# TravisWheelerLab/BATH

Hardware: AMD Instinct MI355X
Metric: DP Gcells/s + residues/s through bathsearch pipeline at 1/2/4/8 MI355X (higher is better)
Workload: dtype u8/i16 integer scores (SSV: exact binary16), f32 Forward

## Files before the change

bath_amd/__init__.py:

```python
import ctypes as C
import os
import subprocess

import numpy as np

_HERE = os.path.dirname(os.path.abspath(__file__))
_ROOT = os.path.dirname(_HERE)
LIB_PATH = os.environ.get("BATH_HIP_LIBRARY") or os.path.join(_HERE, "libbathhip.so")

OK, EINVAL, ERANGE, ENORESULT = 0, 11, 16, 19
KP, K, NEVPARAM = 29, 20, 8
LOGSUM_TABLE, LOGSUM_EXACT, LOGSUM_TABLE_SERIAL, LOGSUM_CONTEXT = 0, 1, 2, 3
LOGSUM_ODDS = 4
ENSEMBLE_SERIAL, ENSEMBLE_STREAMS_HOST, ENSEMBLE_STREAMS_DEVICE = 0, 1, 2
ENSEMBLE_MODES = {"serial": ENSEMBLE_SERIAL, "streams": ENSEMBLE_STREAMS_HOST, "device": ENSEMBLE_STREAMS_DEVICE}
ENS_SAMPLES = 200
ARITH_STRICT, ARITH_ODDS3, ARITH_ODDS = 0, 1, 2
ARITH_MODES = {"strict": ARITH_STRICT, "odds3": ARITH_ODDS3, "odds": ARITH_ODDS}
ENS_OK, ENS_IMPOSSIBLE, ENS_STEP_CAP, ENS_SEG_OVERFLOW = 0, 1, 2, 3
ENS_REGION_OK, ENS_REGION_NO_TRACES = 0, 1

DNA_SYMS = "ACGT-RYMKSWHBVDN*~"
AMINO_SYMS = "ACDEFGHIKLMNPQRSTVWY-BJZOUX*~"

# ... 249 lines not shown
    "bath_hits_count": (C.c_int64, [_vp]),
    "bath_hits_domains": (C.POINTER(FsDomain), [_vp]),
    "bath_hits_cigars": (C.c_void_p, [_vp, _i64p]),
    "bath_hits_traces": (C.c_int, [_vp, C.POINTER(C.POINTER(DomainTrace)), C.POINTER(C.POINTER(C.c_int8)), C.POINTER(_i32p), C.POINTER(_i32p),
                                   C.POINTER(C.POINTER(C.c_int8)), C.POINTER(_f32p)]),
    "bath_tophits_add_serialized": (C.c_int, [_vp, C.c_void_p, C.c_int64, C.c_int64, C.c_int64, C.c_int64, C.POINTER(C.c_char_p), C.POINTER(C.c_char_p),
                                              C.POINTER(C.c_char_p), C.POINTER(C.c_int64)]),
    "bath_dist_shard_range": (None, [C.c_int64, C.c_int, C.c_int, _i64p, _i64p]),
    "bath_dist_items": (C.c_int64, [_i64p, C.POINTER(C.c_double), C.c_int, C.c_int, C.c_int, C.POINTER(DistItem), C.c_int64]),
    "bath_dist_deal": (C.c_int, [C.POINTER(C.c_double), C.c_int64, C.c_int, _i32p]),
    "bath_selftest_cluster_segments": (C.c_int, [C.c_int, _i32p, _i32p, _i32p, _i32p, _i32p, C.c_int, C.c_int, _i32p, C.c_int, _i32p]),
    "bath_selftest_fs_ensemble": (C.c_int, [C.c_int, _f32p, C.c_float, C.c_float, C.c_float, C.c_int, C.c_int, _f32p, _f32p, _i32p, C.c_int, _i32p]),
    "bath_tophits_create": (_vp, []),
    "bath_tophits_destroy": (None, [_vp]),
    "bath_tophits_add": (C.c_int, [_vp, C.POINTER(FsDomain), C.c_int64, C.c_void_p, C.c_int64, C.POINTER(C.c_char_p), C.POINTER(C.c_char_p),
                                   C.POINTER(C.c_char_p), C.POINTER(C.c_int64)]),
    "bath_tophits_finalize": (C.c_int, [_vp, C.c_int64, C.c_int, C.c_double]),
    "bath_tophits_count": (C.c_int64, [_vp]),
    "bath_tophits_reported": (C.c_int64, [_vp]),
    "bath_tophits_get": (C.c_int, [_vp, C.c_int64, C.POINTER(FsDomain), C.POINTER(C.c_int64), C.POINTER(C.c_int32)]),
    "bath_tophits_targets": (C.c_int64, [_vp, C.c_int, C.c_int, C.c_char_p, C.c_int64]),
    "bath_tophits_domain_annotation": (C.c_int64, [_vp, C.c_int64, C.c_int, C.c_int, C.c_char_p, C.c_int64]),
    "bath_tophits_pipeline_statistics": (C.c_int64, [_vp, C.POINTER(PipelineStats), C.POINTER(PipelineParams), C.c_int64, C.c_int64, C.c_int64, C.c_char_p, C.c_int64]),
    "bath_tophits_set_inclusion": (None, [_vp, C.c_double]),
    "bath_tophits_tabular_targets": (C.c_int64, [_vp, C.c_char_p, C.c_char_p, C.c_int, C.c_int, C.c_int, C.c_int, C.c_char_p, C.c_int64]),
    "bath_trace_frameshift_rows": (C.c_int64, [C.POINTER(DomainTrace), C.POINTER(C.c_int8), _i32p, _i32p, C.POINTER(C.c_int8), _u8p, C.c_int32,
                                               C.POINTER(_FsProfile), C.c_int64, C.c_int64, C.POINTER(FsRow), C.c_int64]),
    "bath_tophits_tabular_frameshifts": (C.c_int64, [_vp, C.c_char_p, C.c_char_p, C.POINTER(FsRow), _i64p, C.c_int64, C.c_int, C.c_char_p, C.c_int64]),
    "bath_hip_pipeline_hits": (C.c_int, [_vp, _vp, _vp, C.POINTER(PipelineParams), C.c_double, C.POINTER(PipelineStats),
                                         C.POINTER(C.POINTER(FsDomain)), C.POINTER(C.c_int64), C.POINTER(C.c_int64)]),
    "bath_hip_pipeline_frameshift_domains": (C.c_int, [_vp, _vp, _vp, _vp, _vp, C.POINTER(PipelineParams), C.c_double, C.POINTER(PipelineStats),
                                                      C.POINTER(C.POINTER(FsWindow)), _i64p, C.POINTER(C.POINTER(FsDomain)), _i64p, _i64p]),
    "bath_hip_pipeline_timings": (C.c_int, [_vp, C.c_int, C.POINTER(C.c_char_p), _f32p, _i64p]),
    "bath_hip_fsprofile_convert": (C.c_int, [_vp, C.POINTER(_FsProfile), C.POINTER(_vp)]),
    "bath_hip_fsprofile_destroy": (None, [_vp]),
    "bath_hip_fs3_forward_parser": (C.c_int, [_vp, _vp, _vp, C.c_int, _f32p, _f32p, _i64p]),
    "bath_hip_fs3_backward_parser": (C.c_int, [_vp, _vp, _vp, C.c_int, _f32p, _f32p, _i64p]),
    "bath_hip_vitfilter_bath": (C.c_int, [_vp, _vp, _vp, _f32p, C.c_double, _f32p, _i32p, C.POINTER(C.POINTER(HmmWindow)), _i64p]),
    "bath_hip_ssvfilter_bath": (C.c_int, [_vp, _vp, _vp, C.c_double, C.POINTER(C.POINTER(HmmWindow)), _i64p]),
    "bath_hip_forward_full": (C.c_int, [_vp, _vp, _vp, _i32p, C.c_int, _f32p, _i32p, _f32p, _f32p]),
    "bath_hip_std_envelopes": (C.c_int, [_vp, _vp, _vp, C.POINTER(StdResult), _f32p, _f32p, _f32p, _f32p]),
    "bath_hip_std_envelopes_fill": (C.c_int, [_vp, _vp, _vp, C.POINTER(StdResult), _f32p, _f32p, _f32p, _f32p, C.c_int]),
    "bath_hip_fs5_envelopes_x": (C.c_int, [_vp, _vp, _vp, C.c_int, C.c_int, C.POINTER(Fs5Result), _f32p, _f32p, _f32p, _f32p]),
    "bath_hip_fs5_forward_full": (C.c_int, [_vp, _vp, _vp, C.c_int, _f32p, _f32p, _f32p]),
    "bath_hip_fs5_envelopes": (C.c_int, [_vp, _vp, _vp, C.c_int, C.c_int, C.POINTER(Fs5Result), _f32p, _i64p, _f32p, _i64p]),
    "bath_hip_fs5_forward_parser": (C.c_int, [_vp, _vp, _vp, C.c_int, _f32p]),
    "bath_hip_fs5_forward_parser_odds": (C.c_int, [_vp, _vp, _vp, C.c_int, _f32p]),
    "bath_calib_fit_scores": (C.c_int, [C.POINTER(C.c_uint32), _f32p, C.c_int, C.c_int, C.c_int, _CALIB_SCORE_FN, C.c_void_p, C.c_float,
                                        C.POINTER(C.c_double), C.POINTER(C.c_int)]),
    "bath_hip_calibrate_fs_arith": (C.c_int, [_vp, C.POINTER(_Hmm), C.c_int, C.POINTER(C.c_uint32), C.c_int, C.c_int, C.c_double,
                                              C.POINTER(C.c_double), C.POINTER(C.c_double), C.POINTER(C.c_double), C.POINTER(C.c_double),
                                              C.c_int, C.POINTER(C.c_int)]),
    "bath_calib_sample": (C.c_int, [C.POINTER(C.c_uint32), _f32p, C.c_int, C.c_int, C.c_int, _u8p]),
    "bath_gumbel_fit_complete": (C.c_int, [C.POINTER(C.c_double), C.c_int, C.POINTER(C.c_double), C.POINTER(C.c_double)]),
    "bath_gumbel_invcdf": (C.c_double, [C.c_double, C.c_double, C.c_double]),
    "bath_calib_tau": (C.c_int, [C.POINTER(C.c_double), C.c_int, C.c_double, C.c_double, C.POINTER(C.c_double)]),
    "bath_bg_fs_nullone": (C.c_float, [C.c_int]),
    "bath_hmm_max_length": (C.c_int, [C.POINTER(_Hmm), C.c_double]),
    "bath_hip_calibrate_fs": (C.c_int, [_vp, C.POINTER(_Hmm), C.c_int, C.POINTER(C.c_uint32), C.c_int, C.c_int, C.c_double,
                                        C.POINTER(C.c_double), C.POINTER(C.c_double), C.POINTER(C.c_double), C.POINTER(C.c_double)]),
    "bath_calib_sample_batch": (C.c_int, [C.POINTER(C.c_uint32), _f32p, C.POINTER(C.c_int), C.c_int, C.c_int, C.c_int, _u8p]),
    "bath_hip_calibrate_fs_batch": (C.c_int, [_vp, C.POINTER(C.POINTER(_Hmm)), C.POINTER(C.c_int), C.c_int, C.POINTER(C.c_uint32), C.c_int, C.c_int,
                                              C.c_double, C.POINTER(C.c_double), C.POINTER(C.c_double), C.POINTER(C.c_double), C.POINTER(C.c_double)]),
    "bath_scorematrix_builtin": (C.c_char_p, [C.c_char_p]),
    "bath_scoresystem_create": (C.c_int, [C.c_char_p, C.c_char_p, C.c_double, C.c_double, C.POINTER(_vp), C.c_char_p, C.c_int]),
    "bath_scoresystem_destroy": (None, [_vp]),
# ... 266 lines not shown
            offsets = np.zeros(len(seqs) + 1, dtype=np.int64)
            np.cumsum(lens, out=offsets[1:])
            flat = np.concatenate([np.asarray(s, dtype=np.uint8) for s in seqs]) if len(seqs) else np.zeros(0, np.uint8)
        else:
            flat = np.ascontiguousarray(seqs, dtype=np.uint8)
            offsets = np.ascontiguousarray(offsets, dtype=np.int64)
        if flat.size == 0:
            flat = np.zeros(1, np.uint8)
        self.n = len(offsets) - 1
        self.lengths = np.diff(offsets)
        h = _vp()
        ctx._check(lib().bath_hip_seqs_create(ctx._h, _u8(flat), _i64(offsets), self.n, C.byref(h)), "seqs_create")
        self.ctx, self._h = ctx, h

    def set_context(self, context):
        if context is None:
            self.ctx._check(lib().bath_hip_seqs_set_context(self._h, None), "seqs_set_context")
            return
        c = np.ascontiguousarray(context, dtype=np.int32)
        assert c.shape == (self.n,)
        self.ctx._check(lib().bath_hip_seqs_set_context(self._h, c.ctypes.data_as(C.POINTER(C.c_int32))), "seqs_set_context")

    def read(self):
        L = lib()
        nbytes = L.bath_hip_seqs_read(self._h, None, 0, None, None, None)
        if nbytes < 0:
            self.ctx._check(-1, "seqs_read")
        data = np.zeros(nbytes, np.uint8)
        off, ln, cx = np.zeros(max(self.n, 1), np.int64), np.zeros(max(self.n, 1), np.int32), np.zeros(max(self.n, 1), np.int32)
        if L.bath_hip_seqs_read(self._h, _u8(data), nbytes, _i64(off), ln.ctypes.data_as(_i32p), cx.ctypes.data_as(_i32p)) != nbytes:
            self.ctx._check(-1, "seqs_read")
        return data, off[:self.n], ln[:self.n], cx[:self.n]

    def __del__(self):
        if getattr(self, "_h", None) and getattr(self.ctx, "_h", None):
            lib().bath_hip_seqs_destroy(self._h)
        self._h = None


def pack2(flat, offsets):
    flat = np.ascontiguousarray(flat, dtype=np.uint8)
    offsets = np.ascontiguousarray(offsets, dtype=np.int64)
    lens = np.diff(offsets)
    n = len(lens)
    bad = np.flatnonzero(flat[offsets[0]:offsets[-1]] > 3) + offsets[0]
    seq = np.searchsorted(offsets, bad, side="right") - 1
    pos = (bad - offsets[seq]).astype(np.int32)
    codes = flat[bad].copy()
    if n and (lens == lens[0]).all() and lens[0] % 4 == 0:
        q = (flat[offsets[0]:offsets[-1]] & 3).reshape(-1, 4)
        packed = (q[:, 0] | (q[:, 1] << 2) | (q[:, 2] << 4) | (q[:, 3] << 6)).astype(np.uint8)
    else:
        parts = []
        for i in range(n):
            s = flat[offsets[i]:offsets[i + 1]] & 3
            pad = (-len(s)) % 4
            q = np.concatenate([s, np.zeros(pad, np.uint8)]).reshape(-1, 4)
            parts.append((q[:, 0] | (q[:, 1] << 2) | (q[:, 2] << 4) | (q[:, 3] << 6)).astype(np.uint8))
        packed = np.concatenate(parts) if parts else np.zeros(0, np.uint8)
    return packed, seq.astype(np.int64), pos, codes


class PinnedBuffer:

    def __init__(self, nbytes):
        self.ptr = lib().bath_hip_host_alloc(max(int(nbytes), 1))
# ... 1130 lines not shown
```

bath_amd/csrc/bath_common.hpp:

```cpp
#pragma once
#include <set>
#include <atomic>
#include <hip/hip_runtime.h>

#include <cstdint>
#include <chrono>
#include <cstdio>
#include <cstdlib>
#include <cstring>
#include <condition_variable>
#include <functional>
#include <mutex>
#include <string>
#include <thread>
#include <vector>

#include "bath_hip.h"
#include "bath_tilings.hpp"
#include "bath_slots.hpp"

namespace bath {

inline hipError_t allow_max_lds(const void *fn) {
  static std::mutex mu;
// ... 95 lines not shown
    cv_done.wait(l, [&] { return pending == 0; });
  }
  ~LanePool() {
    { std::lock_guard<std::mutex> l(m); stop = true; }
    cv_work.notify_all();
    for (std::thread &t : th) t.join();
  }
};

struct StageTiming { const char *name; float ms; int64_t launches; };
struct KernelSpan { const char *name; hipEvent_t a, b; double cells, bytes; };

struct PipelineSurvivor {
  int64_t window;
  int64_t aa_off;
  int32_t strand, start;
  int32_t n;
  int32_t win_start = 0;
  int32_t fs_window = -1;
  int64_t fx_off = -1;
};

}

struct bath_hip_ctx;
namespace bath {
extern std::atomic<int> g_ctx_total, g_ctx_internal;
inline int host_contexts() { return g_ctx_total.load() - g_ctx_internal.load(); }
inline void mark_internal(bath_hip_ctx *c);
}
struct bath_hip_ctx {
  int device = 0;
  hipStream_t stream = nullptr;
  hipStream_t tail_stream = nullptr;
  hipStream_t side_stream = nullptr;
  hipEvent_t ev_fork = nullptr, ev_join = nullptr;
  hipStream_t copy_stream = nullptr;
  hipDeviceProp_t prop{};
  int fs_strict = 1;
  int fs_odds = 0;
  int fs5_odds = 0;
  int fs_ensemble = 0;
  std::atomic<int64_t> fs_ens_bound_fallbacks{0}, fs_ens_overflow_fallbacks{0}, fs_ens_bytes_kept{0};
  int std_ensemble = 0;
  std::atomic<int64_t> std_ens_serial_fallbacks{0}, std_ens_twin_fallbacks{0}, std_ens_kernel_regions{0};
  int fs_serial = -1;
  uint64_t tabs_uid = 0;
  const void *tabs_ptr = nullptr;
  uint64_t fsw_pad_uid = 0;
  int orf_tables_id = -1;
  std::string err;
  void set_error(const std::string &m) { err = m; }
  std::vector<float> fsw_len_terms;
  bath::SlotArray<bath::Scratch, bath::DevBuf> scratch;
  bath::SlotArray<bath::Pinned, bath::HostBuf> stage;
  template <class T> int stage_upload(bath::Pinned slot, void *dst, const T *src, size_t n, hipStream_t s) {
    if (stage[slot].reserve(n * sizeof(T) + 64) != hipSuccess) { set_error("cannot allocate page-locked staging memory"); return BATH_EFAIL; }
    std::memcpy(stage[slot].p, src, n * sizeof(T));
    if (hipMemcpyAsync(dst, stage[slot].p, n * sizeof(T), hipMemcpyHostToDevice, s) != hipSuccess) { set_error("staging upload failed"); return BATH_EFAIL; }
    return BATH_OK;
  }
  bath::HostBuf pinned[4];
  bath::HostBuf results_pinned;
  bath_orf_result *d_records = nullptr;
  int64_t n_records = 0;
  std::vector<bath_orf> orfs;
  std::vector<bath_fs_window> fs_windows;
// ... 44 lines not shown
  }
  void span_end(int idx, hipStream_t s) { if (idx >= 0) (void)hipEventRecord(spans[(size_t)idx].b, s); }
  std::vector<bath_hip_ctx *> lanes;
  bath::LanePool *lane_pool = nullptr;
  hipEvent_t ev_lanes = nullptr;
  bath_hip_ctx *aux = nullptr;
  bath_hip_ctx *aux2 = nullptr;
  bath_hip_ctx *aux3 = nullptr;
  bool internal = false;
};

namespace bath {
inline void mark_internal(bath_hip_ctx *c) { if (c && !c->internal) { c->internal = true; g_ctx_internal.fetch_add(1); } }
}

struct SeqView {
  const uint8_t *data;
  const int64_t *off;
  const int32_t *len;
  int64_t n;
  const int32_t *context;
};

struct bath_hip_seqs {
  bath_hip_ctx *ctx = nullptr;
  int64_t n = 0;
  int64_t total = 0;
  int64_t total_aligned = 0;
  mutable int64_t cache_minlen = -1, cache_nres = 0, cache_max_orfs = 0;
  mutable int64_t ntiles = -1;
  mutable void *d_tile_desc = nullptr;
  mutable int32_t *d_tile_first = nullptr;
  bool is_part = false;
  int64_t first_window = 0;
  mutable std::vector<bath_hip_seqs *> parts;
  int32_t maxlen = 0;
  uint8_t *d_data = nullptr;
  int64_t *d_off = nullptr;
  int32_t *d_len = nullptr;
  int32_t *d_context = nullptr;
  uint8_t *d_packed = nullptr;
  int64_t *d_poff = nullptr;
  int64_t packed_bytes = 0;
  void *d_exc = nullptr;
  int64_t exc_cap = 0, n_exc = 0;
  hipEvent_t ev_upload = nullptr;
  bool upload_pending = false;
  std::vector<int64_t> h_off;
  std::vector<int32_t> h_len;
  std::vector<int32_t> h_context;
  SeqView view() const { return SeqView{d_data, d_off, d_len, n, d_context}; }
};

struct LenTables {
  int32_t maxL = -1;
  uint8_t *d_tjb = nullptr;
  int16_t *d_xwmove = nullptr;
  float   *d_pmove = nullptr;
  float   *d_nullsc = nullptr;
  float   *d_lt1 = nullptr;
  float   *d_lt2 = nullptr;
  float   *d_p1 = nullptr;
  std::vector<uint8_t> h_tjb;
  std::vector<int16_t> h_xwmove;
  std::vector<float> h_pmove, h_nullsc;
};
// ... 66 lines not shown
```

bath_amd/csrc/bath_launch.hpp:

```cpp
#pragma once
#include <utility>

#include "bath_common.hpp"

namespace bath {

struct Cand {
  int64_t *window;  int32_t *sf;
  int32_t *startj;  int32_t *len;
  int16_t *v;
  int64_t *off;
  int32_t *msv_status, *vit_status, *fwd_status, *stage, *flags;
  float *usc, *nullsc, *filtersc, *vfsc, *fwdsc;
  double *P;
  int32_t *kminmax;
};

int build_orf_records(bath_hip_ctx *ctx, const Cand &cand, int nc, int64_t window_offset, bath_orf_result **d_out, int64_t *n_out);

struct VitWindowArgs {
  double invP_vit, invP_msv;
  const float *d_filtersc;
  const uint8_t *d_ssv_scores;
  void *d_wins;
  int *d_win_count;
  int win_cap;
  int32_t *d_kminmax;
};

int ssv_table_fits(bath_hip_ctx *ctx, const bath_hip_oprofile *om);
int launch_ssv_lane(bath_hip_ctx *ctx, const bath_hip_oprofile *om, SeqView v, const int32_t *d_order, int16_t *d_v);
int launch_ssv_classify(bath_hip_ctx *ctx, const bath_hip_oprofile *om, int64_t n, const int32_t *d_len, const int16_t *d_v, float *d_sc, int32_t *d_status);
int launch_msv_wave(bath_hip_ctx *ctx, const bath_hip_oprofile *om, SeqView v, const int32_t *d_todo, int64_t ntodo, float *d_sc, int32_t *d_status, const int *ntodo_dev, bool lane_ok = true);
int launch_msv_lane(bath_hip_ctx *ctx, const bath_hip_oprofile *om, SeqView v, const int32_t *d_todo, int64_t ntodo, float *d_sc, int32_t *d_status, const int *ntodo_dev);
bool msv_stage_supported(const bath_hip_oprofile *om);
int launch_vit_wave(bath_hip_ctx *ctx, const bath_hip_oprofile *om, SeqView v, const int32_t *d_todo, int64_t ntodo, float *d_sc, int32_t *d_status,
                    const VitWindowArgs *wa, const int *ntodo_dev);
int launch_fwd_wave(bath_hip_ctx *ctx, const bath_hip_oprofile *om, SeqView v, const int32_t *d_todo, int64_t ntodo, float *d_sc, int32_t *d_status, const int *ntodo_dev,
                    float *d_xmx = nullptr, const int64_t *d_xmx_off = nullptr, float *d_dp = nullptr, const int64_t *d_dp_off = nullptr, int unihit = 0,
                    const int32_t *d_cfg_len = nullptr);
int launch_bwd_wave(bath_hip_ctx *ctx, const bath_hip_oprofile *om, SeqView v, int64_t n, const float *d_fwd_xmx, const int64_t *d_xmx_off,
                    float *d_sc, int32_t *d_status, float *d_bck_xmx, float *d_dp = nullptr, const int64_t *d_dp_off = nullptr, int unihit = 0);
int launch_bias_lane(bath_hip_ctx *ctx, const bath_hip_oprofile *om, SeqView v, const float *d_eo, int eo_stride, const int32_t *d_todo, int64_t ntodo,
                     float *d_nullsc, float *d_filtersc);

int vit_lane_supported(const bath_hip_oprofile *om);
int launch_len_sort(bath_hip_ctx *ctx, const int32_t *d_todo, const int *d_ntodo, const int32_t *d_len, int *d_bins, int32_t *d_sorted);
int launch_vit_lane(bath_hip_ctx *ctx, const bath_hip_oprofile *om, SeqView v, const int32_t *d_todo, int64_t ntodo, const int *ntodo_dev,
                    float *d_sc, int32_t *d_status, const VitWindowArgs *wa, const int *skip_dev = nullptr);
const int *len_sort_count_longer(const int *d_bins, int T);
int64_t lane_min_nt();
const char *vit_lane_kernel_name(const bath_hip_oprofile *om);
int launch_vit_sorted(bath_hip_ctx *ctx, const bath_hip_oprofile *om, SeqView v, const int32_t *d_todo, int64_t cap, const int *d_ntodo, const int32_t *d_len,
                      int *d_bins, int32_t *d_sorted, float *d_sc, int32_t *d_status, const VitWindowArgs *wa, const std::function<int(hipStream_t)> &beside);
struct MsvConsts;
MsvConsts msv_consts(const bath_hip_oprofile *om);

int pipeline_filters_survivors(bath_hip_ctx *ctx, const bath_hip_oprofile *om, const bath_hip_seqs *dna, const bath_pipeline_params *prm,
                               bath_pipeline_stats *stats, std::vector<PipelineSurvivor> *out, const uint8_t **d_pool);

struct FsWinDev {
  int64_t src_off;
  int64_t dst_off;
  int32_t seq_n, start, len, strand, kmin, kmax;
};
int fs_gather_view(bath_hip_ctx *ctx, const bath_hip_seqs *dna, std::vector<FsWinDev> &regs, const uint8_t *d_comp, bath_hip_seqs *view, const FsWinDev **d_desc_out);

struct WindowRec;
struct FsCandRec { int64_t window, aa_off; double P; int32_t cand, sf, startj, len; float fwdsc, nullsc; int64_t fxoff; };
struct FsLaneSurv {
  const FsCandRec *d_c; const WindowRec *d_w;
  int32_t n_c, n_w, cand_base;
  int64_t first_window, dpool;
};
struct FsOrfDev {
  int64_t w, aa_off; double P;
  int32_t cand, strand, start, end, n; float fwd_null;
  int32_t wb, we;
  int32_t dw_n, dw_len, dw_k;
  int32_t kmin, kmax;
  int32_t g0, g1;
  int32_t pad_;
};
struct FsWinBuild {
  int32_t n_orfs = 0, nw = 0, maxlen = 0;
// ... 120 lines not shown
```

bath_amd/csrc/bath_pipeline.hip:

```cpp
#include <algorithm>
#include <cmath>
#include <cstring>
#include <cstdlib>
#include <map>
#include <thread>

#include "bath_common.hpp"
#include "bath_kernels.hpp"
#include "bath_launch.hpp"
#include "host_model.hpp"

using namespace bath;

namespace bath {

static const double kLog2 = 0.69314718055994529;

enum { FLAG_VIT_RUN = 1, FLAG_HAS_WIN = 2 };

struct Counters {
  int cand_count, todo_msv, todo_vit, todo_ssvb, todo_vit2, todo_fwd, win_count, overflow;
  int todo_lb, pad_;
  unsigned long long n_orfs, orf_res;
  unsigned long long n_past_msv, n_past_bias, n_past_vit, n_past_fwd;
  unsigned long long pos_past_msv, pos_past_bias, pos_past_vit, pos_past_fwd;
  unsigned long long res_vit, res_fwd;
  unsigned long long res_seen;
};

struct Params {
  double F1, F2, F3, F4;
  int do_bias, fs_pipe, minlen;
  float evparam[BATH_NEVPARAM];
};

template <int NR, int G>
__global__ __launch_bounds__(256, NR <= 76 ? 4 : 1) void ssv_orf_kernel(const uint8_t *__restrict__ aa, const OrfRec *__restrict__ orfs, const int *__restrict__ n_orfs_dev,
                                                      SeqView dna, const int16_t *__restrict__ cost_tab, int row_bytes,
// ... 662 lines not shown
struct FilterState {
  PipelineWork W;
  Counters hc{};
  const uint8_t *d_ssvsc = nullptr;
  const float *d_bgf = nullptr;
  OrfTablesDev tt{};
};
}

__global__ __launch_bounds__(64) void fwd_keep_offsets_kernel(const int32_t *__restrict__ todo, const int *__restrict__ ntodo_dev, const int32_t *__restrict__ len,
                                                              int64_t *__restrict__ off, int64_t cap) {
  const int lane = threadIdx.x, n = *ntodo_dev;
  int64_t base = 0;
  for (int j0 = 0; j0 < n; j0 += 64) {
    const int j = j0 + lane;
    const int sid = j < n ? todo[j] : -1;
    const int64_t v = sid >= 0 ? ((int64_t)len[sid] + 1) * 6 : 0;
    int64_t incl = v;
    for (int d = 1; d < 64; d <<= 1) { const int64_t u = __shfl_up(incl, d, 64); if (lane >= d) incl += u; }
    if (sid >= 0) off[sid] = (base + incl <= cap) ? base + incl - v : (int64_t)-1;
    base += __shfl(incl, 63, 64);
  }
}

static int cascade_model_ok(bath_hip_ctx *ctx, const bath_hip_oprofile *om) {
  if (om->M <= kCascadeMaxNodes) return BATH_OK;
  ctx->set_error("the filter cascade supports models up to " + std::to_string(kCascadeMaxNodes) + " nodes (this one has " + std::to_string(om->M) + ")");
  return BATH_EINVAL;
}

static int launch_ssv_bath(bath_hip_ctx *ctx, hipStream_t stream, const bath_hip_oprofile *om, const Cand &cand, Counters *ctr, const int32_t *todo, const uint8_t *pool,
                           const uint8_t *ssv_scores, const MsvConsts &mc, double invP, WindowRec *wins, int win_cap);

static int run_filters(bath_hip_ctx *ctx, const bath_hip_oprofile *om, const bath_hip_seqs *dna,
                       const bath_pipeline_params *prm, bath_pipeline_stats *stats,
                       const bath_orf_result **results, int64_t *n_results, FilterState *state) {
  if (!ctx || !om || !dna || !prm) return BATH_EINVAL;
  if (cascade_model_ok(ctx, om) != BATH_OK) return BATH_EINVAL;
  BATH_HIP_TRY(ctx, hipSetDevice(ctx->device));
  if (n_results) *n_results = 0;
  if (results) *results = nullptr;
  if (stats) std::memset(stats, 0, sizeof *stats);
  const int64_t nwin = dna->n;
  if (nwin == 0) return BATH_OK;
  const int M = om->M;
  const int max_orf = dna->maxlen / 3 + 1;
  int st = om->ensure_len_tables(max_orf);
  if (st != BATH_OK) return st;

  OrfTablesDev tt{};
  if (prm->strands < 0 || prm->strands > 2 || prm->initiator < 0 || prm->initiator > 2) { ctx->set_error("bath_pipeline_params: strands / initiator out of range"); return BATH_EINVAL; }
  if ((st = orf_tables_upload(ctx, prm->ncbi_table, &tt, prm->initiator)) != BATH_OK) return st;
  if ((st = ensure_emit_table(ctx, om, prm->F1, max_orf)) != BATH_OK) return st;
  DevBuf &b_tabs = ctx->scratch[Scratch::kSsvScoreTable], &b_work = ctx->scratch[Scratch::kCascadeWork];
  const size_t ssv_bytes = (size_t)(M + 1) * kKp;
  const size_t tabs_bytes = 8192 + ssv_bytes + 256 + 20 * 4 + 256;
  if (tabs_bytes > b_tabs.cap) ctx->tabs_uid = 0;
  BATH_HIP_TRY(ctx, b_tabs.reserve(tabs_bytes));
  char *tp = b_tabs.as<char>();
  const int16_t *d_emit = om->d_emit;
  uint8_t *d_ssvsc = reinterpret_cast<uint8_t *>(tp); tp += (ssv_bytes + 255) / 256 * 256;
  float *d_bgf = reinterpret_cast<float *>(tp);
  if (ctx->tabs_uid != om->uid || ctx->tabs_ptr != b_tabs.p) {
    std::vector<uint8_t> ssv_scores(ssv_bytes, 0);
    bath_hip_oprofile_get_ssv_scores(om, ssv_scores.data());
    BATH_HIP_TRY(ctx, hipMemcpyAsync(d_ssvsc, ssv_scores.data(), ssv_scores.size(), hipMemcpyHostToDevice, ctx->stream));
// ... 40 lines not shown
  BATH_HIP_TRY(ctx, b_orfs.reserve((size_t)(max_orfs + 64) * sizeof(OrfRec)));
  BATH_HIP_TRY(ctx, b_misc.reserve((5 * nent + kOrfMiscInts) * sizeof(int32_t)));
  OrfBuffers ob{};
  orf_buffers_carve(&ob, b_aa.p, b_slots.p, b_orfs.p, b_misc.p, nent);

  const int NRk = om->NR;
  const size_t ssv_shmem = (size_t)kSsvRows * om->ssv_row_bytes;
  if ((st = ssv_table_fits(ctx, om)) != BATH_OK) return st;
  const int dec_blocks = ctx->prop.multiProcessorCount * 4;

  std::vector<hipEvent_t> &ev = ctx->ev_pool;
  while (ev.size() < 12) { hipEvent_t e; BATH_HIP_TRY(ctx, hipEventCreate(&e)); ev.push_back(e); }

  PipelineWork W;
  Counters hc{};
  int win_need = 0;
  for (int attempt = 0;; attempt++) {
    size_t need = layout(W, nullptr, (int)cap, win_need);
    BATH_HIP_TRY(ctx, b_work.reserve(need + 4096));
    layout(W, b_work.as<char>(), (int)cap, win_need);
    W.pool = b_aa.as<uint8_t>();
    BATH_HIP_TRY(ctx, hipMemsetAsync(W.ctr, 0, sizeof(Counters), ctx->stream));
    SeqView cv{W.pool, W.cand.off, W.cand.len, cap};

    int e = 0;
    BATH_HIP_TRY(ctx, hipEventRecord(ev[e++], ctx->stream));
    if ((st = launch_orf_scan(ctx, dna, tt, prm->min_orf_len, ob, &W.ctr->n_orfs, &W.ctr->orf_res, prm->strands)) != BATH_OK) return st;
    BATH_HIP_TRY(ctx, hipEventRecord(ev[e++], ctx->stream));
    {
      static const int ssv_chunk = [] { const char *e = std::getenv("BATH_HIP_SSV_CHUNK"); return e ? std::atoi(e) : 0; }();
      int blocks = ctx->prop.multiProcessorCount * 4;
      const int ssv_threads = 256;
      const int wpb = ssv_threads / 64;
      if (ssv_chunk > 0) blocks = (int)std::min<int64_t>((max_orfs + (int64_t)wpb * (64 / om->G) * ssv_chunk - 1) / ((int64_t)wpb * (64 / om->G) * ssv_chunk), 1 << 30);
      bool launched = false;
#define BATH_ORF_CASE(N, GG)                                                                                                     \
  if (!launched && NRk == N && om->G == GG) {                                                                                    \
    if (ssv_shmem > 64 * 1024) (void)bath::allow_max_lds((const void *)ssv_orf_kernel<N, GG>); \
    hipLaunchKernelGGL((ssv_orf_kernel<N, GG>), dim3(blocks), dim3(ssv_threads), ssv_shmem, ctx->stream, W.pool, ob.sorted, ob.ntotal,                  \
                       dna->view(), om->d_ssv, om->ssv_row_bytes, d_emit, max_orf, W.cand, W.cand_cap, W.ctr, ssv_chunk);        \
    launched = true;                                                                                                             \
  }
      BATH_SSV_SHAPES(BATH_ORF_CASE)
#undef BATH_ORF_CASE
      if (!launched) { ctx->set_error("SSV kernel: no tile shape for this model length"); return BATH_EINVAL; }
      BATH_HIP_TRY(ctx, hipGetLastError());
    }
    BATH_HIP_TRY(ctx, hipEventRecord(ev[e++], ctx->stream));
    hipStream_t bulk_stream = ctx->stream;
    struct StreamRestore { bath_hip_ctx *c; hipStream_t s; ~StreamRestore() { c->stream = s; } } stream_restore{ctx, bulk_stream};
    if (ctx->tail_stream) {
      BATH_HIP_TRY(ctx, hipStreamWaitEvent(ctx->tail_stream, ev[e - 1], 0));
      ctx->stream = ctx->tail_stream;
    }
    const bool few_cands = dna->total < lane_min_nt(), few_msv = dna->total < 2 * lane_min_nt();
    const F1Tables f1t{om->d_bias_eo, om->lt.d_nullsc, om->lt.d_p1, om->lt.d_lt1, om->lt.d_lt2};
    const bool msv_stage = !few_msv && msv_stage_supported(om);
    if (msv_stage) {
      bool launched = false;
#define BATH_MSV_STAGE_CASE(N, ...)                                                                                                         \
  if (!launched && NRk == N) {                                                                                                              \
    hipLaunchKernelGGL((msv_stage_kernel<N>), dim3((unsigned)((W.cand_cap + 255) / 256)), dim3(256), ssv_shmem, ctx->stream, W.cand, W.cand_cap, W.ctr, om->d_msv, \
                       om->ssv_row_bytes, om->lt.d_tjb, mc, P, W.pool, M, f1t, W.todo_vit, W.todo_ssvb);                                      \
    launched = true;                                                                                                                        \
  }
      BATH_MSV_LANE_NR(BATH_MSV_STAGE_CASE)
#undef BATH_MSV_STAGE_CASE
      if (!launched) { ctx->set_error("MSV stage kernel: no tile shape for this model length"); return BATH_EINVAL; }
      BATH_HIP_TRY(ctx, hipGetLastError());
      BATH_HIP_TRY(ctx, hipEventRecord(ev[e++], ctx->stream));
      BATH_HIP_TRY(ctx, hipEventRecord(ev[e++], ctx->stream));
// ... 67 lines not shown
      BATH_HIP_TRY(ctx, hipEventElapsedTime(&ms, ev[i], ev[i + 1]));
      ctx->timings.push_back(StageTiming{names[i], ms, launches[i]});
    }
    break;
  }

  if (stats) {
    stats->nres = nres; stats->n_orfs = (int64_t)hc.n_orfs;
    stats->n_past_msv = (int64_t)hc.n_past_msv; stats->n_past_bias = (int64_t)hc.n_past_bias;
    stats->n_past_vit = (int64_t)hc.n_past_vit; stats->n_past_fwd = (int64_t)hc.n_past_fwd;
    stats->pos_past_msv = (int64_t)hc.pos_past_msv; stats->pos_past_bias = (int64_t)hc.pos_past_bias;
    stats->pos_past_vit = (int64_t)hc.pos_past_vit; stats->pos_past_fwd = (int64_t)hc.pos_past_fwd;
    stats->cells_msv = (int64_t)(hc.orf_res - hc.res_seen) * M; stats->cells_vit = (int64_t)hc.res_vit * M; stats->cells_fwd = (int64_t)hc.res_fwd * M;
  }

  if (results) {
    bath_orf_result *d_rec = nullptr;
    int64_t nrec = 0;
    if (dna->n > (int64_t)UINT32_MAX || dna->maxlen / 3 >= (1 << 28)) { ctx->set_error("block too large for the ORF records' sort key (2^32 windows, 805 Mnt per window)"); return BATH_ERANGE; }
    if ((st = build_orf_records(ctx, W.cand, hc.cand_count, dna->is_part ? dna->first_window : 0, &d_rec, &nrec)) != BATH_OK) return st;
    ctx->d_records = d_rec; ctx->n_records = nrec;
    if (!dna->is_part) {
      BATH_HIP_TRY(ctx, ctx->results_pinned.reserve((size_t)std::max<int64_t>(nrec, 1) * sizeof(bath_orf_result)));
      if (nrec > 0) BATH_HIP_TRY(ctx, hipMemcpyAsync(ctx->results_pinned.p, d_rec, (size_t)nrec * sizeof(bath_orf_result), hipMemcpyDeviceToHost, ctx->stream));
      BATH_HIP_TRY(ctx, hipStreamSynchronize(ctx->stream));
      *results = ctx->results_pinned.as<bath_orf_result>();
    } else *results = nullptr;
    if (n_results) *n_results = nrec;
  } else if (n_results) *n_results = (int64_t)hc.n_past_msv;
  if (state) { state->W = W; state->hc = hc; state->d_ssvsc = d_ssvsc; state->d_bgf = d_bgf; state->tt = tt; }
  return BATH_OK;
}

static int pipeline_lane_count(const bath_hip_seqs *dna) {
  const char *e = std::getenv("BATH_HIP_LANES");
  const int forced = e ? std::atoi(e) : 0;
  if (forced > 0) return (int)std::min<int64_t>(forced, std::max<int64_t>(dna->n, 1));
  if (dna->is_part || dna->n < 8) return 1;
  int K = (dna->total >= ((int64_t)1 << 28)) ? 2 : 1;
  const int64_t by_size = (dna->total + ((int64_t)1 << 34) - 1) >> 34;
  if (by_size > K) K = (int)std::min<int64_t>(by_size, std::max<int64_t>(dna->n, 1));
  return K;
}

static int ensure_parts(bath_hip_ctx *ctx, const bath_hip_seqs *dna, int K) {
  if ((int)dna->parts.size() == K) return BATH_OK;
  for (bath_hip_seqs *p : dna->parts) bath_hip_seqs_destroy(p);
  dna->parts.clear();
  int64_t w0 = 0;
  for (int k = 0; k < K; k++) {
    static const double split2 = [] { const char *e = std::getenv("BATH_HIP_LANE_SPLIT"); const double v = e ? std::atof(e) : 0.0; return (v > 0.05 && v < 0.95) ? v : 0.5; }();
    int64_t w1 = w0;
    if (k == K - 1) w1 = dna->n;
    else {
      const int64_t target = (K == 2) ? (int64_t)((double)dna->total_aligned * split2) : dna->total_aligned / K * (k + 1);
      w1 = std::lower_bound(dna->h_off.begin() + w0, dna->h_off.end(), target) - dna->h_off.begin();
      w1 = std::max(w1, std::min(w0 + 1, dna->n));
    }
    bath_hip_seqs *p = new bath_hip_seqs();
    p->ctx = ctx; p->is_part = true; p->first_window = w0; p->n = w1 - w0;
    const int64_t base = w0 < dna->n ? dna->h_off[(size_t)w0] : dna->total_aligned;
    p->h_off.resize((size_t)p->n); p->h_len.assign(dna->h_len.begin() + w0, dna->h_len.begin() + w1);
    for (int64_t i = 0; i < p->n; i++) {
      p->h_off[(size_t)i] = dna->h_off[(size_t)(w0 + i)] - base;
      p->maxlen = std::max(p->maxlen, p->h_len[(size_t)i]);
      p->total += p->h_len[(size_t)i];
    }
    p->total_aligned = (w1 < dna->n ? dna->h_off[(size_t)w1] : dna->total_aligned) - base;
    p->d_data = dna->d_data + base;
    p->d_len = dna->d_len + w0;
    if (dna->d_context) { p->d_context = dna->d_context + w0; p->h_context.assign(dna->h_context.begin() + w0, dna->h_context.begin() + w1); }
    dna->parts.push_back(p);
    if (hipMalloc((void **)&p->d_off, (size_t)std::max<int64_t>(p->n, 1) * sizeof(int64_t)) != hipSuccess) { ctx->set_error("hipMalloc (block parts)"); return BATH_EMEM; }
    if (p->n > 0 && hipMemcpy(p->d_off, p->h_off.data(), (size_t)p->n * sizeof(int64_t), hipMemcpyHostToDevice) != hipSuccess) { ctx->set_error("hipMemcpy (block parts)"); return BATH_EFAIL; }
    w0 = w1;
  }
  return BATH_OK;
}

template <class After>
static int run_filters_lanes(bath_hip_ctx *ctx, const bath_hip_oprofile *om, const bath_hip_seqs *dna,
                             const bath_pipeline_params *prm, bath_pipeline_stats *stats,
                             const bath_orf_result **results, int64_t *n_results, std::vector<FilterState> *states, After after) {
  if (!ctx || !om || !dna || !prm) return BATH_EINVAL;
  if (cascade_model_ok(ctx, om) != BATH_OK) return BATH_EINVAL;
  const int K = pipeline_lane_count(dna);
  if (K <= 1) {
    states->assign(1, FilterState{});
    int st = run_filters(ctx, om, dna, prm, stats, results, n_results, &(*states)[0]);
    if (st != BATH_OK) return st;
    return after(0, ctx, dna, (*states)[0]);
  }
  BATH_HIP_TRY(ctx, hipSetDevice(ctx->device));
  int st = om->ensure_len_tables(dna->maxlen / 3 + 1);
  if (st != BATH_OK) return st;
  if ((st = ensure_emit_table(ctx, om, prm->F1, dna->maxlen / 3 + 1)) != BATH_OK) return st;
  while ((int)ctx->lanes.size() < K) {
    bath_hip_ctx *lane = nullptr;
    if ((st = bath_hip_init(ctx->device, &lane)) != BATH_OK) { ctx->set_error("cannot create a pipeline lane"); return st; }
    mark_internal(lane);
    const char *pe = std::getenv("BATH_HIP_LANE_PRIO");
    if (!(pe && pe[0] == '0')) {
      int lo = 0, hi = 0;
      if (hipDeviceGetStreamPriorityRange(&lo, &hi) == hipSuccess && lo != hi) {
        (void)hipStreamDestroy(lane->stream);
        const char *te = std::getenv("BATH_HIP_TAIL_PRIO");
        const bool tails = te && te[0] == '1';
        const int prio = tails ? (ctx->lanes.empty() ? std::min(lo, hi + 1) : lo) : (ctx->lanes.empty() ? hi : lo);
        if (hipStreamCreateWithPriority(&lane->stream, hipStreamNonBlocking, prio) != hipSuccess) { ctx->set_error("hipStreamCreateWithPriority"); return BATH_EFAIL; }
        if (tails && hipStreamCreateWithPriority(&lane->tail_stream, hipStreamNonBlocking, hi) != hipSuccess) { ctx->set_error("hipStreamCreateWithPriority"); return BATH_EFAIL; }
      }
    }
    ctx->lanes.push_back(lane);
  }
  for (bath_hip_ctx *lane : ctx->lanes) { lane->fs_strict = ctx->fs_strict; lane->fs_odds = ctx->fs_odds; lane->fs5_odds = ctx->fs5_odds; }
  if ((st = ensure_parts(ctx, dna, K)) != BATH_OK) return st;
  std::vector<bath_pipeline_stats> pst((size_t)K);
  std::vector<const bath_orf_result *> pres((size_t)K, nullptr);
  std::vector<int64_t> pn((size_t)K, 0);
  std::vector<int> rc((size_t)K, BATH_OK);
  states->assign((size_t)K, FilterState{});
  if (!ctx->ev_lanes) BATH_HIP_TRY(ctx, hipEventCreateWithFlags(&ctx->ev_lanes, hipEventDisableTiming));
  BATH_HIP_TRY(ctx, hipEventRecord(ctx->ev_lanes, ctx->stream));
  for (int k = 0; k < K; k++) BATH_HIP_TRY(ctx, hipStreamWaitEvent(ctx->lanes[(size_t)k]->stream, ctx->ev_lanes, 0));
  if (!ctx->lane_pool) ctx->lane_pool = new LanePool();
  ctx->lane_pool->run(K, [&](int k) {
    bath_hip_ctx *lane = ctx->lanes[(size_t)k];
    rc[(size_t)k] = run_filters(lane, om, dna->parts[(size_t)k], prm, &pst[(size_t)k], results ? &pres[(size_t)k] : nullptr, &pn[(size_t)k], &(*states)[(size_t)k]);
    if (rc[(size_t)k] == BATH_OK) rc[(size_t)k] = after(k, lane, dna->parts[(size_t)k], (*states)[(size_t)k]);
  });
  for (int k = 0; k < K; k++)
    if (rc[(size_t)k] != BATH_OK) { ctx->set_error(ctx->lanes[(size_t)k]->err); return rc[(size_t)k]; }

  bath_pipeline_stats tot{};
  int64_t ntot = 0;
  for (int k = 0; k < K; k++) {
    const bath_pipeline_stats &a = pst[(size_t)k];
    tot.nres += a.nres; tot.n_orfs += a.n_orfs; tot.n_past_msv += a.n_past_msv; tot.n_past_bias += a.n_past_bias; tot.n_past_vit += a.n_past_vit;
    tot.n_past_fwd += a.n_past_fwd; tot.pos_past_msv += a.pos_past_msv; tot.pos_past_bias += a.pos_past_bias; tot.pos_past_vit += a.pos_past_vit;
    tot.pos_past_fwd += a.pos_past_fwd; tot.cells_msv += a.cells_msv; tot.cells_vit += a.cells_vit; tot.cells_fwd += a.cells_fwd;
    ntot += pn[(size_t)k];
  }
  if (stats) *stats = tot;
  if (results) {
    BATH_HIP_TRY(ctx, ctx->results_pinned.reserve((size_t)std::max<int64_t>(ntot, 1) * sizeof(bath_orf_result)));
    bath_orf_result *dst = ctx->results_pinned.as<bath_orf_result>();
// ... 495 lines not shown
```

bath_amd/csrc/bath_viterbi.hip:

```cpp
#include <algorithm>
#include <cstdlib>
#include <functional>

#include "bath_common.hpp"
#include "bath_kernels.hpp"
#include "bath_launch.hpp"

using namespace bath;

namespace bath {

__device__ __forceinline__ s16x2 pk_adds(s16x2 a, s16x2 b) { return __builtin_elementwise_add_sat(a, b); }
__device__ __forceinline__ s16x2 pk_max(s16x2 a, s16x2 b) { return __builtin_elementwise_max(a, b); }
__device__ __forceinline__ s16x2 as_s2(unsigned v) { return __builtin_bit_cast(s16x2, v); }
__device__ __forceinline__ unsigned as_u(s16x2 v) { return __builtin_bit_cast(unsigned, v); }

struct VitLaneTables {
  const int16_t *rw;
  int rw_pitch_bytes;
  const uint32_t *tw2;
  const int16_t *rank;
};

struct VitLaneConsts {
// ... 253 lines not shown
  c.M = om->M; c.base_w = om->base_w; c.xwE_loop = om->xw_E[0]; c.xwE_move = om->xw_E[1]; c.Q8 = std::max(2, ((om->M - 1) / 8) + 1);
  c.scale_w = om->scale_w; c.scale_b = om->scale_b; c.base_b = om->base_b; c.tec_b = om->tec_b; c.bias_b = om->bias_b;
  const float *fsc = nullptr; const uint8_t *ssv = nullptr; WindowRec *wins = nullptr; int *wc = nullptr; int cap = 0; int32_t *kmm = nullptr;
  if (wa) { c.invP_vit = wa->invP_vit; c.invP_msv = wa->invP_msv; fsc = wa->d_filtersc; ssv = wa->d_ssv_scores; wins = (WindowRec *)wa->d_wins; wc = wa->d_win_count; cap = wa->win_cap; kmm = wa->d_kminmax; }
  const int NRv = om->vit_NR;
  const size_t shmem = (size_t)30 * om->vit_rw_pitch + (size_t)2 * NRv * 2 + 16;
  const int blocks = (int)((ntodo + 255) / 256);
  bool launched = false;
#define BATH_VITL_CASE(N, ...)                                                                                                         \
  if (!launched && NRv == N) {                                                                                                         \
    hipLaunchKernelGGL(vit_lane_kernel<N>, dim3(blocks), dim3(256), shmem, ctx->stream, v, tb, tb.tw2, c, om->lt.d_xwmove, om->lt.d_tjb, d_todo, ntodo, \
                       ntodo_dev, skip_dev, d_sc, d_status, fsc, ssv, wins, wc, cap, kmm);                                                       \
    launched = true;                                                                                                                   \
  }
  BATH_VIT_LANE_NR(BATH_VITL_CASE)
#undef BATH_VITL_CASE
  if (!launched) { ctx->set_error("lane-per-target Viterbi kernel: unsupported model length"); return BATH_EINVAL; }
  BATH_HIP_TRY(ctx, hipGetLastError());
  return BATH_OK;
}

int64_t lane_min_nt() {
  static const int64_t v = [] { const char *e = std::getenv("BATH_HIP_LANE_MIN_NT"); return e ? std::atoll(e) : (int64_t)150'000'000; }();
  return v;
}

const char *vit_lane_kernel_name(const bath_hip_oprofile *om) {
#define BATH_VITL_NAME(N, ...) if (om->vit_NR == N) return "vit_lane_kernel<" #N ">";
  BATH_VIT_LANE_NR(BATH_VITL_NAME)
#undef BATH_VITL_NAME
  return "vit_lane_kernel<?>";
}

int launch_vit_sorted(bath_hip_ctx *ctx, const bath_hip_oprofile *om, SeqView v, const int32_t *d_todo, int64_t cap, const int *d_ntodo, const int32_t *d_len,
                      int *d_bins, int32_t *d_sorted, float *d_sc, int32_t *d_status, const VitWindowArgs *wa, const std::function<int(hipStream_t)> &beside) {
  int st;
  if ((st = launch_len_sort(ctx, d_todo, d_ntodo, d_len, d_bins, d_sorted)) != BATH_OK) return st;
  if (!ctx->side_stream) {
    BATH_HIP_TRY(ctx, hipStreamCreateWithFlags(&ctx->side_stream, hipStreamNonBlocking));
    BATH_HIP_TRY(ctx, hipEventCreateWithFlags(&ctx->ev_fork, hipEventDisableTiming));
    BATH_HIP_TRY(ctx, hipEventCreateWithFlags(&ctx->ev_join, hipEventDisableTiming));
  }
  static const int long_orf = [] { const char *e = std::getenv("BATH_HIP_VIT_LONG"); return e ? std::atoi(e) : kVitLongTarget; }();
  const int *d_nlong = len_sort_count_longer(d_bins, long_orf);
  BATH_HIP_TRY(ctx, hipEventRecord(ctx->ev_fork, ctx->stream));
  BATH_HIP_TRY(ctx, hipStreamWaitEvent(ctx->side_stream, ctx->ev_fork, 0));
  {
    hipStream_t main_stream = ctx->stream;
    ctx->stream = ctx->side_stream;
    st = launch_vit_wave(ctx, om, v, d_sorted, cap, d_sc, d_status, wa, d_nlong);
    ctx->stream = main_stream;
    if (st != BATH_OK) return st;
    if (beside && (st = beside(ctx->side_stream)) != BATH_OK) return st;
  }
  BATH_HIP_TRY(ctx, hipEventRecord(ctx->ev_join, ctx->side_stream));
  if ((st = launch_vit_lane(ctx, om, v, d_sorted, cap, d_ntodo, d_sc, d_status, wa, d_nlong)) != BATH_OK) return st;
  BATH_HIP_TRY(ctx, hipStreamWaitEvent(ctx->stream, ctx->ev_join, 0));
  return BATH_OK;
}

}
```

include/bath_hip.h:

```cpp
#ifndef BATH_HIP_H
#define BATH_HIP_H

#include <stdint.h>
#include <stddef.h>

#ifdef __cplusplus
extern "C" {
#endif

#define BATH_OK          0
#define BATH_EFAIL       1
#define BATH_EMEM        5
#define BATH_EFORMAT     7
#define BATH_EINVAL     11
#define BATH_ERANGE     16
#define BATH_ENORESULT  19
#define BATH_ENODEVICE  40

#define BATH_KP_AMINO   29
#define BATH_K_AMINO    20
#define BATH_KP_DNA     18
#define BATH_NEVPARAM    8
#define BATH_FTAU        4
#define BATH_FLAMBDA     5
// ... 174 lines not shown
} bath_orf_result;

typedef struct {
  int64_t nres, n_orfs;
  int64_t n_past_msv, n_past_bias, n_past_vit, n_past_fwd;
  int64_t pos_past_msv, pos_past_bias, pos_past_vit, pos_past_fwd;
  int64_t cells_msv, cells_vit, cells_fwd;
} bath_pipeline_stats;

typedef struct {
  int64_t window;
  int32_t strand, frame;
  int32_t start, end;
  int32_t n;
  int64_t aa_off;
} bath_orf;
int  bath_hip_translate_orfs(bath_hip_ctx *ctx, const bath_hip_seqs *dna, int ncbi_table, int min_orf_len,
                             const bath_orf **orfs, int64_t *n_orfs, const uint8_t **aa);
int  bath_hip_translate_orfs_opts(bath_hip_ctx *ctx, const bath_hip_seqs *dna, int ncbi_table, int min_orf_len, int strands, int initiator,
                                  const bath_orf **orfs, int64_t *n_orfs, const uint8_t **aa);
typedef struct {
  int64_t aa_off;
  int32_t window;
  int32_t len_sf;
} bath_orf_work;
int  bath_hip_orf_worklist(bath_hip_ctx *ctx, const bath_orf_work **list, int64_t *n);
int  bath_gencode_initiators(int ncbi_table, int initiator, uint8_t is_init[64]);

void bath_pipeline_params_default(bath_pipeline_params *p, int fs_pipe);
int  bath_hip_pipeline_filters(bath_hip_ctx *ctx, const bath_hip_oprofile *om, const bath_hip_seqs *dna,
                               const bath_pipeline_params *params, bath_pipeline_stats *stats,
                               const bath_orf_result **results, int64_t *n_results);
int  bath_hip_pipeline_timings(const bath_hip_ctx *ctx, int max, const char **names, float *ms, int64_t *launches);

typedef struct {
  const char *name;
  float   ms;
  int64_t launches;
  double  cells, bytes;
} bath_kernel_time;
int  bath_hip_kernel_times(bath_hip_ctx *ctx, int max, bath_kernel_time *out);

typedef struct {
  int64_t window;
  int32_t strand;
  int32_t n, length;
  int32_t orf_cnt, k_min, k_max;
  float   tot_orfsc;
  float   nullsc, filtersc, fwdsc;
  double  P_tot, P_min, P_fs, P_null;
  int32_t branch;
} bath_fs_window;
int  bath_hip_pipeline_frameshift(bath_hip_ctx *ctx, const bath_hip_oprofile *om, const bath_hip_fsprofile *om_fs3,
                                  const bath_hip_seqs *dna, const bath_pipeline_params *params, bath_pipeline_stats *stats,
                                  const bath_orf_result **results, int64_t *n_results,
                                  const bath_fs_window **fs_windows, int64_t *n_fs_windows);

typedef struct {
  int64_t window;
  int32_t strand;
  int32_t fs_window;
  int32_t ienv, jenv, iali, jali;
  int32_t ihmm, jhmm;
  float   envsc, oasc;
  float   domcorrection, dombias;
  float   bitscore, pre_score;
// ... 238 lines not shown
```

Baseline: 214.7 billion.

## Add filler lane with register-sized SSV grid and per-lane stream priorities

When the pipeline runs three lanes, the third partition becomes a filler whose SSV grid is sized from the register headroom left by the Viterbi lane kernel, so it can co-reside on CUs alongside the other lanes' work. Lane shares become configurable per lane (defaulting to 0.47/0.47 for three lanes), and stream priorities are assigned after all lanes exist, with graded priority per lane index and the last lane lowest. The aim is to fill idle CU capacity left by the long-tail Viterbi work. The risk is contention with the main lanes and a hard failure if the runtime does not report register counts. A parts query is also exposed to Python.

```diff
diff --git a/bath_amd/__init__.py b/bath_amd/__init__.py
--- a/bath_amd/__init__.py
+++ b/bath_amd/__init__.py
@@ -305,6 +305,7 @@
     "bath_hip_pipeline_frameshift_domains": (C.c_int, [_vp, _vp, _vp, _vp, _vp, C.POINTER(PipelineParams), C.c_double, C.POINTER(PipelineStats),
                                                       C.POINTER(C.POINTER(FsWindow)), _i64p, C.POINTER(C.POINTER(FsDomain)), _i64p, _i64p]),
     "bath_hip_pipeline_timings": (C.c_int, [_vp, C.c_int, C.POINTER(C.c_char_p), _f32p, _i64p]),
+    "bath_hip_pipeline_parts": (C.c_int, [_vp, C.c_int, _i64p, _i64p]),
     "bath_hip_fsprofile_convert": (C.c_int, [_vp, C.POINTER(_FsProfile), C.POINTER(_vp)]),
     "bath_hip_fsprofile_destroy": (None, [_vp]),
     "bath_hip_fs3_forward_parser": (C.c_int, [_vp, _vp, _vp, C.c_int, _f32p, _f32p, _i64p]),
@@ -637,6 +638,11 @@
             self.ctx._check(-1, "seqs_read")
         return data, off[:self.n], ln[:self.n], cx[:self.n]
 
+    def parts(self):
+        first, n = np.zeros(64, np.int64), np.zeros(64, np.int64)
+        k = lib().bath_hip_pipeline_parts(self._h, 64, _i64(first), _i64(n))
+        return [(int(first[i]), int(n[i])) for i in range(k)]
+
     def __del__(self):
         if getattr(self, "_h", None) and getattr(self.ctx, "_h", None):
             lib().bath_hip_seqs_destroy(self._h)
diff --git a/bath_amd/csrc/bath_common.hpp b/bath_amd/csrc/bath_common.hpp
--- a/bath_amd/csrc/bath_common.hpp
+++ b/bath_amd/csrc/bath_common.hpp
@@ -151,7 +151,8 @@
 struct bath_hip_ctx {
   int device = 0;
   hipStream_t stream = nullptr;
-  hipStream_t tail_stream = nullptr;
+  bool stream_has_prio = false;
+  int stream_prio = 0;  hipStream_t tail_stream = nullptr;
   hipStream_t side_stream = nullptr;
   hipEvent_t ev_fork = nullptr, ev_join = nullptr;
   hipStream_t copy_stream = nullptr;
@@ -262,6 +263,7 @@
   mutable void *d_tile_desc = nullptr;
   mutable int32_t *d_tile_first = nullptr;
   bool is_part = false;
+  bool is_filler = false;
   int64_t first_window = 0;
   mutable std::vector<bath_hip_seqs *> parts;
   int32_t maxlen = 0;
diff --git a/bath_amd/csrc/bath_launch.hpp b/bath_amd/csrc/bath_launch.hpp
--- a/bath_amd/csrc/bath_launch.hpp
+++ b/bath_amd/csrc/bath_launch.hpp
@@ -51,6 +51,8 @@
 const int *len_sort_count_longer(const int *d_bins, int T);
 int64_t lane_min_nt();
 const char *vit_lane_kernel_name(const bath_hip_oprofile *om);
+int kernel_wave_regs(const void *fn);
+int vit_lane_kernel_regs(const bath_hip_oprofile *om);
 int launch_vit_sorted(bath_hip_ctx *ctx, const bath_hip_oprofile *om, SeqView v, const int32_t *d_todo, int64_t cap, const int *d_ntodo, const int32_t *d_len,
                       int *d_bins, int32_t *d_sorted, float *d_sc, int32_t *d_status, const VitWindowArgs *wa, const std::function<int(hipStream_t)> &beside);
 struct MsvConsts;
diff --git a/bath_amd/csrc/bath_pipeline.hip b/bath_amd/csrc/bath_pipeline.hip
--- a/bath_amd/csrc/bath_pipeline.hip
+++ b/bath_amd/csrc/bath_pipeline.hip
@@ -3,7 +3,9 @@
 #include <cstring>
 #include <cstdlib>
 #include <map>
+#include <mutex>
 #include <thread>
+#include <utility>
 
 #include "bath_common.hpp"
 #include "bath_kernels.hpp"
@@ -732,6 +734,21 @@
 static int launch_ssv_bath(bath_hip_ctx *ctx, hipStream_t stream, const bath_hip_oprofile *om, const Cand &cand, Counters *ctr, const int32_t *todo, const uint8_t *pool,
                            const uint8_t *ssv_scores, const MsvConsts &mc, double invP, WindowRec *wins, int win_cap);
 
+static int ssv_fill_blocks(const bath_hip_oprofile *om, const void *ssv_fn) {
+  static const int forced = [] { const char *e = std::getenv("BATH_HIP_SSV_FILL_BLOCKS"); return e ? std::atoi(e) : 0; }();
+  if (forced > 0) return std::min(forced, 4);
+  static std::mutex mu;
+  static std::map<std::pair<const void *, int>, int> known;
+  std::lock_guard<std::mutex> lock(mu);
+  const auto key = std::make_pair(ssv_fn, (int)om->vit_NR);
+  auto it = known.find(key);
+  if (it == known.end()) {
+    const int vit = vit_lane_kernel_regs(om), ssv = kernel_wave_regs(ssv_fn);
+    it = known.emplace(key, (vit < 1 || ssv < 1) ? -1 : std::min(4, std::max(1, (512 - vit) / ssv))).first;
+  }
+  return it->second;
+}
+
 static int run_filters(bath_hip_ctx *ctx, const bath_hip_oprofile *om, const bath_hip_seqs *dna,
                        const bath_pipeline_params *prm, bath_pipeline_stats *stats,
                        const bath_orf_result **results, int64_t *n_results, FilterState *state) {
@@ -838,11 +855,18 @@
       int blocks = ctx->prop.multiProcessorCount * 4;
       const int ssv_threads = 256;
       const int wpb = ssv_threads / 64;
+      const bool filler = dna->is_filler && vit_lane_supported(om) && ssv_chunk <= 0;
       if (ssv_chunk > 0) blocks = (int)std::min<int64_t>((max_orfs + (int64_t)wpb * (64 / om->G) * ssv_chunk - 1) / ((int64_t)wpb * (64 / om->G) * ssv_chunk), 1 << 30);
       bool launched = false;
 #define BATH_ORF_CASE(N, GG)                                                                                                     \
   if (!launched && NRk == N && om->G == GG) {                                                                                    \
-    if (ssv_shmem > 64 * 1024) (void)bath::allow_max_lds((const void *)ssv_orf_kernel<N, GG>); \
+    const void *ssv_fn = (const void *)ssv_orf_kernel<N, GG>;                                                                    \
+    if (ssv_shmem > 64 * 1024) (void)bath::allow_max_lds(ssv_fn);                                                                \
+    if (filler) {                                                                                                                \
+      const int per_cu = ssv_fill_blocks(om, ssv_fn);                                                                            \
+      if (per_cu < 1) { ctx->set_error("SSV filler grid: the runtime does not report the kernels' register counts"); return BATH_EFAIL; } \
+      blocks = ctx->prop.multiProcessorCount * per_cu;                                                                           \
+    }                                                                                                                            \
     hipLaunchKernelGGL((ssv_orf_kernel<N, GG>), dim3(blocks), dim3(ssv_threads), ssv_shmem, ctx->stream, W.pool, ob.sorted, ob.ntotal,                  \
                        dna->view(), om->d_ssv, om->ssv_row_bytes, d_emit, max_orf, W.cand, W.cand_cap, W.ctr, ssv_chunk);        \
     launched = true;                                                                                                             \
@@ -976,6 +1000,8 @@
   return BATH_OK;
 }
 
+constexpr double kFillerFirstShare = 0.47, kFillerSecondShare = 0.47;
+
 static int pipeline_lane_count(const bath_hip_seqs *dna) {
   const char *e = std::getenv("BATH_HIP_LANES");
   const int forced = e ? std::atoi(e) : 0;
@@ -987,22 +1013,51 @@
   return K;
 }
 
+static std::vector<double> part_shares(int K) {
+  static const std::vector<double> given = [] {
+    std::vector<double> v;
+    const char *e = std::getenv("BATH_HIP_LANE_SPLIT");
+    while (e && *e) {
+      char *end = nullptr;
+      v.push_back(std::strtod(e, &end));
+      if (end == e) { v.clear(); break; }
+      e = (*end == ',') ? end + 1 : end;
+      if (*end != ',' && *end != '\0') { v.clear(); break; }
+    }
+    return v;
+  }();
+  if (K == 2 && given.size() == 1) return {(given[0] > 0.05 && given[0] < 0.95) ? given[0] : 0.5};
+  if (K >= 3 && (int)given.size() == K - 1) {
+    double sum = 0.0;
+    bool ok = true;
+    for (double s : given) { ok = ok && s > 0.01; sum += s; }
+    if (ok && sum < 0.99) return given;
+  }
+  if (K == 2) return {0.5};
+  if (K == 3) return {kFillerFirstShare, kFillerSecondShare};
+  return {};
+}
+
 static int ensure_parts(bath_hip_ctx *ctx, const bath_hip_seqs *dna, int K) {
   if ((int)dna->parts.size() == K) return BATH_OK;
   for (bath_hip_seqs *p : dna->parts) bath_hip_seqs_destroy(p);
   dna->parts.clear();
+  const std::vector<double> shares = part_shares(K);
   int64_t w0 = 0;
+  double upto = 0.0;
   for (int k = 0; k < K; k++) {
-    static const double split2 = [] { const char *e = std::getenv("BATH_HIP_LANE_SPLIT"); const double v = e ? std::atof(e) : 0.0; return (v > 0.05 && v < 0.95) ? v : 0.5; }();
     int64_t w1 = w0;
     if (k == K - 1) w1 = dna->n;
     else {
-      const int64_t target = (K == 2) ? (int64_t)((double)dna->total_aligned * split2) : dna->total_aligned / K * (k + 1);
+      if (!shares.empty()) upto += shares[(size_t)k];
+      const int64_t target = !shares.empty() ? (int64_t)((double)dna->total_aligned * upto) : dna->total_aligned / K * (k + 1);
       w1 = std::lower_bound(dna->h_off.begin() + w0, dna->h_off.end(), target) - dna->h_off.begin();
       w1 = std::max(w1, std::min(w0 + 1, dna->n));
+      w1 = std::max(w0, std::min(w1, dna->n - (K - 1 - k)));
     }
     bath_hip_seqs *p = new bath_hip_seqs();
     p->ctx = ctx; p->is_part = true; p->first_window = w0; p->n = w1 - w0;
+    p->is_filler = K == 3 && k == 2;
     const int64_t base = w0 < dna->n ? dna->h_off[(size_t)w0] : dna->total_aligned;
     p->h_off.resize((size_t)p->n); p->h_len.assign(dna->h_len.begin() + w0, dna->h_len.begin() + w1);
     for (int64_t i = 0; i < p->n; i++) {
@@ -1020,6 +1075,13 @@
     w0 = w1;
   }
   return BATH_OK;
+}
+
+extern "C" int bath_hip_pipeline_parts(const bath_hip_seqs *dna, int max, int64_t *first_window, int64_t *n_windows) {
+  if (!dna || !first_window || !n_windows) return 0;
+  const int n = std::min<int>(max, (int)dna->parts.size());
+  for (int i = 0; i < n; i++) { first_window[i] = dna->parts[(size_t)i]->first_window; n_windows[i] = dna->parts[(size_t)i]->n; }
+  return n;
 }
 
 template <class After>
@@ -1043,19 +1105,25 @@
     bath_hip_ctx *lane = nullptr;
     if ((st = bath_hip_init(ctx->device, &lane)) != BATH_OK) { ctx->set_error("cannot create a pipeline lane"); return st; }
     mark_internal(lane);
-    const char *pe = std::getenv("BATH_HIP_LANE_PRIO");
-    if (!(pe && pe[0] == '0')) {
-      int lo = 0, hi = 0;
-      if (hipDeviceGetStreamPriorityRange(&lo, &hi) == hipSuccess && lo != hi) {
+    ctx->lanes.push_back(lane);
+  }
+  {
+    static const bool prio_on = [] { const char *pe = std::getenv("BATH_HIP_LANE_PRIO"); return !(pe && pe[0] == '0'); }();
+    static const bool tails = [] { const char *te = std::getenv("BATH_HIP_TAIL_PRIO"); return te && te[0] == '1'; }();
+    int lo = 0, hi = 0;
+    if (prio_on && hipDeviceGetStreamPriorityRange(&lo, &hi) == hipSuccess && lo != hi) {
+      for (int k = 0; k < K; k++) {
+        bath_hip_ctx *lane = ctx->lanes[(size_t)k];
+        const int prio = tails ? (k == 0 ? std::min(lo, hi + 1) : lo) : (k == K - 1 ? lo : std::min(lo, hi + k));
+        if (lane->stream_has_prio && lane->stream_prio == prio) continue;
+        (void)hipStreamSynchronize(lane->stream);
         (void)hipStreamDestroy(lane->stream);
-        const char *te = std::getenv("BATH_HIP_TAIL_PRIO");
-        const bool tails = te && te[0] == '1';
-        const int prio = tails ? (ctx->lanes.empty() ? std::min(lo, hi + 1) : lo) : (ctx->lanes.empty() ? hi : lo);
+        lane->stream = nullptr;
         if (hipStreamCreateWithPriority(&lane->stream, hipStreamNonBlocking, prio) != hipSuccess) { ctx->set_error("hipStreamCreateWithPriority"); return BATH_EFAIL; }
-        if (tails && hipStreamCreateWithPriority(&lane->tail_stream, hipStreamNonBlocking, hi) != hipSuccess) { ctx->set_error("hipStreamCreateWithPriority"); return BATH_EFAIL; }
+        lane->stream_has_prio = true; lane->stream_prio = prio;
+        if (tails && !lane->tail_stream && hipStreamCreateWithPriority(&lane->tail_stream, hipStreamNonBlocking, hi) != hipSuccess) { ctx->set_error("hipStreamCreateWithPriority"); return BATH_EFAIL; }
       }
     }
-    ctx->lanes.push_back(lane);
   }
   for (bath_hip_ctx *lane : ctx->lanes) { lane->fs_strict = ctx->fs_strict; lane->fs_odds = ctx->fs_odds; lane->fs5_odds = ctx->fs5_odds; }
   if ((st = ensure_parts(ctx, dna, K)) != BATH_OK) return st;
diff --git a/bath_amd/csrc/bath_viterbi.hip b/bath_amd/csrc/bath_viterbi.hip
--- a/bath_amd/csrc/bath_viterbi.hip
+++ b/bath_amd/csrc/bath_viterbi.hip
@@ -309,6 +309,19 @@
   return "vit_lane_kernel<?>";
 }
 
+int kernel_wave_regs(const void *fn) {
+  hipFuncAttributes at{};
+  if (hipFuncGetAttributes(&at, fn) != hipSuccess) { (void)hipGetLastError(); return -1; }
+  return at.numRegs > 0 ? (at.numRegs + 7) / 8 * 8 : -1;
+}
+
+int vit_lane_kernel_regs(const bath_hip_oprofile *om) {
+#define BATH_VITL_REGS(N, ...) if (om->vit_NR == N) return kernel_wave_regs((const void *)vit_lane_kernel<N>);
+  BATH_VIT_LANE_NR(BATH_VITL_REGS)
+#undef BATH_VITL_REGS
+  return -1;
+}
+
 int launch_vit_sorted(bath_hip_ctx *ctx, const bath_hip_oprofile *om, SeqView v, const int32_t *d_todo, int64_t cap, const int *d_ntodo, const int32_t *d_len,
                       int *d_bins, int32_t *d_sorted, float *d_sc, int32_t *d_status, const VitWindowArgs *wa, const std::function<int(hipStream_t)> &beside) {
   int st;
diff --git a/include/bath_hip.h b/include/bath_hip.h
--- a/include/bath_hip.h
+++ b/include/bath_hip.h
@@ -230,6 +230,7 @@
                                const bath_pipeline_params *params, bath_pipeline_stats *stats,
                                const bath_orf_result **results, int64_t *n_results);
 int  bath_hip_pipeline_timings(const bath_hip_ctx *ctx, int max, const char **names, float *ms, int64_t *launches);
+int  bath_hip_pipeline_parts(const bath_hip_seqs *dna, int max, int64_t *first_window, int64_t *n_windows);
 
 typedef struct {
   const char *name;
```

Result: slower. 211.5 billion (-1.5%).
